# ETH3D/badslam

Measured on AMD Instinct MI355X. Metric: BA iterations/sec (and ms/iter) at N keyframes x M surfels, 640x480, higher is better.
Workload: dtype f32

## Files before the change

badslam_amd/capi.py:

```python
import ctypes as C
import os

_HERE = os.path.dirname(os.path.abspath(__file__))
LIB_PATH = os.path.join(os.environ.get("BADSLAM_LIB_DIR") or os.path.join(_HERE, "lib"), "libbadslam_hip.so")

SURFEL_ATTRIBUTE_COUNT = 17
MERGE_BUFFER_COUNT = 3
KF_ACTIVE, KF_COVISIBLE_ACTIVE, KF_INACTIVE = 0, 1, 2
ARITHMETIC_EXACT, ARITHMETIC_FAST = 0, 1

SURFEL_X, SURFEL_Y, SURFEL_Z, SURFEL_NORMAL, SURFEL_RADIUS_SQUARED, SURFEL_COLOR, SURFEL_DESCRIPTOR1, SURFEL_DESCRIPTOR2 = range(8)
SURFEL_ACCUM0 = 8


class BackendError(RuntimeError):
    pass


class Camera(C.Structure):
    _fields_ = [("fx", C.c_float), ("fy", C.c_float), ("cx", C.c_float), ("cy", C.c_float),
                ("width", C.c_int32), ("height", C.c_int32)]


class DepthParams(C.Structure):
# ... 170 lines not shown
                                            C.POINTER(Cost)]),
    "bahip_debug_set_cost_shape": (C.c_int, [C.c_int, C.c_int, C.c_int, C.c_int]),
    "bahip_debug_evaluate_pairs": (C.c_int, [C.c_void_p, C.POINTER(Frame), C.POINTER(C.c_float), C.POINTER(Surfels),
                                             C.POINTER(C.c_uint32), C.c_int, C.POINTER(C.c_float)]),
    "bahip_debug_read_pcg_vector": (C.c_int, [C.c_void_p, C.c_int, C.c_size_t, C.c_size_t, C.POINTER(C.c_float)]),
    "bahip_gather_surfel_shards": (C.c_int, [C.c_void_p, C.POINTER(Surfels), C.c_uint32, C.c_int, C.c_int, C.c_uint32, C.POINTER(Surfels),
                                             C.POINTER(C.c_uint32), C.POINTER(C.c_uint32)]),
    "bahip_extract_surfel_shard": (C.c_int, [C.c_void_p, C.POINTER(Surfels), C.c_int, C.c_int, C.c_uint32, C.POINTER(Surfels), C.POINTER(C.c_uint32)]),
    "bahip_debug_set_intrinsics_bin_capacity": (C.c_int, [C.c_void_p, C.c_int]),
    "bahip_debug_intrinsics_bin_stats": (C.c_int, [C.c_void_p, C.POINTER(C.c_uint32), C.POINTER(C.c_uint32), C.POINTER(C.c_uint64)]),
    "bahip_debug_set_intrinsics_slices": (C.c_int, [C.c_void_p, C.c_int]),
    "bahip_debug_read_intrinsics_sums": (C.c_int, [C.c_void_p, C.POINTER(C.c_float), C.POINTER(C.c_float)]),
    "bahip_exchange_stats": (C.c_int, [C.c_void_p, C.POINTER(C.c_longlong), C.POINTER(C.c_longlong), C.c_int]),
    "bahip_context_set_lifecycle_dealing": (C.c_int, [C.c_void_p, C.c_int]),
    "bahip_debug_lifecycle_deal_stats": (C.c_int, [C.c_void_p, C.POINTER(C.c_longlong), C.c_int]),
    "bahip_debug_exact_sum": (C.c_int, [C.c_void_p, C.POINTER(C.c_float), C.c_size_t, C.c_int, C.POINTER(C.c_double)]),
    "bahip_debug_count_pairs": (C.c_int, [C.c_void_p, C.POINTER(Surfels), C.POINTER(C.c_uint64)]),
    "bahip_debug_set_launch_shapes": (C.c_int, [C.c_int, C.c_int]),
    "bahip_debug_set_pose_form": (C.c_int, [C.c_int]),
    "bahip_debug_set_append_groups": (C.c_int, [C.c_int]),
    "bahip_debug_geometry_hybrid_launches": (C.c_int, [C.POINTER(C.c_longlong)]),
    "bahip_debug_set_creation_chain": (C.c_int, [C.c_int]),
    "bahip_debug_creation_chain_batches": (C.c_int, [C.POINTER(C.c_longlong)]),
    "bahip_debug_set_merge_cells": (C.c_int, [C.c_int]),
    "bahip_debug_merge_cells_batches": (C.c_int, [C.POINTER(C.c_longlong)]),
    "bahip_debug_set_pose_lds_items": (C.c_int, [C.c_int]),
    "bahip_debug_set_pose_lds_shape": (C.c_int, [C.c_int, C.c_int]),
    "bahip_debug_set_fused_iteration_begin": (C.c_int, [C.c_int]),
    "bahip_debug_set_intrinsics_reduce_form": (C.c_int, [C.c_int]),
    "bahip_debug_set_pose_rounds_ahead": (C.c_int, [C.c_int]),
    "bahip_debug_set_device_loop": (C.c_int, [C.c_int]),
    "bahip_debug_alternating_loop_calls": (C.c_int, [C.POINTER(C.c_longlong), C.POINTER(C.c_longlong)]),
    "bahip_debug_set_pcg_lds_form": (C.c_int, [C.c_int]),
    "bahip_debug_pose_form_launches": (C.c_int, [C.POINTER(C.c_longlong), C.POINTER(C.c_longlong), C.c_int]),
    "bahip_debug_pose_kernel_dispatches": (C.c_int, [C.POINTER(C.c_longlong)]),
    "bahip_debug_pcg_step1_form_launches": (C.c_int, [C.POINTER(C.c_longlong), C.POINTER(C.c_longlong)]),
    "bahip_debug_pose_limbs": (C.c_int, [C.c_void_p, C.POINTER(C.c_float), C.c_size_t, C.POINTER(C.c_longlong)]),
    "bahip_debug_jacobian": (C.c_int, [C.c_void_p, C.c_int, C.POINTER(C.c_float), C.c_int, C.POINTER(C.c_float), C.c_int]),
    "bahip_debug_read_pattern": (C.c_int, [C.c_void_p, C.c_size_t, C.c_int, C.c_int]),
    "bahip_debug_exact_math": (C.c_int, [C.c_void_p, C.c_int, C.POINTER(C.c_float), C.POINTER(C.c_float), C.c_size_t]),
    "bahip_debug_pose_step": (C.c_int, [C.c_void_p, C.POINTER(C.c_float), C.POINTER(C.c_float), C.POINTER(C.c_float)]),
    "bahip_debug_wave_reduce": (C.c_int, [C.c_void_p, C.POINTER(C.c_float), C.POINTER(C.c_float)]),
    "bahip_last_stage_time_ms": (C.c_int, [C.c_void_p, C.c_int, C.POINTER(C.c_float), C.POINTER(C.c_int)]),
    "bahip_set_profiling": (C.c_int, [C.c_void_p, C.c_int]),
    "bahip_frame_planes_create": (C.c_int, [C.c_void_p, C.c_int, C.c_int, C.c_int, C.c_int, C.POINTER(C.c_void_p)]),
    "bahip_frame_planes_update": (C.c_int, [C.c_void_p, C.c_void_p, C.POINTER(Frame)]),
    "bahip_frame_planes_destroy": (None, [C.c_void_p]),
    "bahip_stage_work_units": (C.c_int, [C.c_void_p, C.c_int, C.POINTER(C.c_longlong)]),
}

_lib = None


def load():
    global _lib
    if _lib is None:
        if not os.path.exists(LIB_PATH):
            raise BackendError(
                f"{LIB_PATH} not found: build the HIP extension first (python -c 'import __graft_entry__ as g; g.build()'). "
                "There is no CPU fallback.")
        lib = C.CDLL(LIB_PATH)
        for name, (restype, argtypes) in SIGNATURES.items():
            if os.environ.get("BADSLAM_LIB_DIR") and not hasattr(lib, name):
                continue
            fn = getattr(lib, name)
            fn.restype = restype
# ... 9 lines not shown
```

badslam_amd/csrc/ba_launch.h:

```cpp
#pragma once

#include "ba_device.h"
#include <cstdlib>

inline int bahip_env_int(const char* name, int fallback) {
  const char* e = std::getenv(name);
  return e ? std::atoi(e) : fallback;
}

#ifdef BAHIP_FAST_MATH
#define BAHIP_FLAVOUR fast
#else
#define BAHIP_FLAVOUR exact
#endif
#define BAHIP_FLAVOURED_BEGIN namespace bahip { namespace BAHIP_FLAVOUR {
#define BAHIP_FLAVOURED_END } }

namespace bahip {

struct SupportingView {
  uint32_t* b[BAHIP_MERGE_BUFFER_COUNT];
  uint32_t pitch;
};

// ... 49 lines not shown
bool launch_tile_order(hipStream_t stream, uint32_t* tile_cost, uint32_t padded_tiles, uint32_t* sched);
struct PoseLoopControl {
  int* ctl = nullptr;
  int* host_ctl = nullptr;
  int phase_end = 0;
  int iteration = 0;
  int min_iterations = 0;
  int* round_log = nullptr;
  int log_slot = 0;
  int publish = 1;
  int next_mode = -1;
  const uint8_t* in_window = nullptr;
  const int* covis_offsets = nullptr;
  const int* covis_indices = nullptr;
};
void launch_pose_solve(hipStream_t stream, void* work, int num_work, HbFixed* Hb, KfEntry* frames, int write_back,
                       int update_activation, int round, void* host_out,
                       int sequence ,
                       const PoseLoopControl* loop = nullptr);
void launch_pose_init_from_keyframes(hipStream_t stream, const KfEntry* frames, int num_kfs, void* work, HbFixed* Hb, void* host_out,
                                     int kf_rank = 0, int kf_world = 1 ,
                                     const int* stop = nullptr);

void launch_window_activation(hipStream_t stream, KfEntry* frames, int num_kfs, const uint8_t* in_window, const int* offsets,
                              const int* indices, const int* stop = nullptr);
void launch_propagate_covisible(hipStream_t stream, KfEntry* frames, int num_kfs, const int* offsets, const int* indices,
                                const int* stop = nullptr);
bool launch_iteration_begin(hipStream_t stream, KfEntry* frames, int num_kfs, int mode, const uint8_t* in_window, const int* offsets, const int* indices,
                            void* work, HbFixed* Hb, void* host_out, const int* stop);

void set_tile_waves(int waves);
long long geometry_hybrid_launches();
void set_pose_lds_waves(int waves);
void set_pose_lds_parts_shift(int shift);
void set_pose_lds_items(int items);
void pcg_step1_form_launches(long long out[2]);
long long pose_kernel_dispatches();
void pose_form_launches(long long out[2], bool reset);
void set_pose_form(int form);
void set_pose_parts(int parts);
void launch_jacobian_debug(hipStream_t stream, int kind, const float* in, float* out);
void launch_pose_step_debug(hipStream_t stream, const float* in, float* out);
void launch_exact_math_debug(hipStream_t stream, int kind, const float* in, float* out, size_t n);
void launch_pose_limbs_debug(hipStream_t stream, const float* in, long long* out, size_t n);
void launch_wave_reduce_debug(hipStream_t stream, const float* in, float* out);
void launch_evaluate_pairs(hipStream_t stream, const Intrinsics& in, const KfEntry& frame, const SurfelsView& s,
                           const uint32_t* indices, int count, float* out);

struct IntrBins {
  uint32_t* cursors;
  uint32_t* records;
  uint32_t capacity;
  int bins_x;
};
int intrinsics_bin_count(const Intrinsics& in, int* bins_x_out);
size_t intrinsics_bin_record_bytes();
void launch_intrinsics_accumulate(hipStream_t st, bool depth, bool color, const Intrinsics& in, const KfEntry* kfs, int num_kfs,
                                  const SurfelsView& s, double* glob, double* cells, const IntrBins& bins, const uint32_t* sched,
                                  uint32_t position_begin = 0, uint32_t position_count = 0 ,
                                  int classes = 1 ,
                                  int kf_rank = 0, int kf_world = 1 );
uint32_t intrinsics_sweep_positions(uint32_t surfels, const uint32_t* sched);
void launch_intrinsics_bin_reduce(hipStream_t st, bool depth, const Intrinsics& in, const SurfelsView& s, double* cells, const IntrBins& bins);
void set_intrinsics_reduce_form(int form);
size_t intrinsics_schur_partials(int S);
void launch_intrinsics_finish(hipStream_t st, bool schur, int S, const double* glob_d, const double* cells_d, float* glob_f, float* cells_f,
// ... 140 lines not shown
void launch_delete_unpack(hipStream_t st, const SurfelsView& s, const void* packed);
void launch_shard_to_cloud(hipStream_t st, const SurfelsView& shard, const SurfelsView& cloud, uint32_t rank, uint32_t world, uint32_t chunk);
void launch_cloud_to_shard(hipStream_t st, const SurfelsView& cloud, const SurfelsView& shard, uint32_t rank, uint32_t world, uint32_t chunk);
size_t sort_scratch_bytes(uint32_t n);
hipError_t sort_surfels_spatially(hipStream_t st, const SurfelsView& s, float inv_cell, void* scratch, size_t scratch_bytes);
size_t scan_temp_bytes(size_t n);
hipError_t scan_flags_inclusive(hipStream_t st, void* temp, size_t temp_bytes, const uint8_t* flags, uint32_t* out, int n);
hipError_t scan_u32_exclusive(hipStream_t st, void* temp, size_t temp_bytes, const uint32_t* in, uint32_t* out, int n);
hipError_t launch_compact(hipStream_t st, const SurfelsView& s, uint32_t* invalid, uint32_t* free_rank, uint32_t* free_list,
                          uint32_t surfel_count, void* temp, size_t temp_bytes);


#define BAHIP_FLAVOURED_DECLARATIONS                                                                                                          \
                                                                                                                      \
  void launch_activation(hipStream_t stream, const Intrinsics& in, const KfEntry* kfs, int num_kfs, const SurfelsView& s, uint32_t surfels_size); \
  void launch_normals(hipStream_t stream, const Intrinsics& in, const KfEntry* kfs, int num_kfs, const SurfelsView& s);                       \
  void launch_geometry(hipStream_t stream, bool use_depth, bool use_desc, const Intrinsics& in, const KfEntry* kfs, int num_kfs,              \
                       const SurfelsView& s, long long activate_count, const uint32_t* sched, const int* stop);                              \
  void launch_geometry_phase(hipStream_t stream, int phase, bool use_depth, bool use_desc, const Intrinsics& in, const KfEntry* kfs,          \
                             int num_kfs, const SurfelsView& s, long long activate_count, const ClassPartials& cpn, const ClassPartials& cpp); \
  void launch_activation_hits(hipStream_t stream, const Intrinsics& in, const KfEntry* kfs, int num_kfs, const SurfelsView& s,                \
                              uint32_t surfels_size, int kf_rank, int kf_world, uint32_t* hits);                                              \
  void launch_normals_phase(hipStream_t stream, int phase, const Intrinsics& in, const KfEntry* kfs, int num_kfs, const SurfelsView& s,      \
                            const ClassPartials& cp);                                                                                         \
  void set_tile_waves(int waves);                                                                                                             \
  long long geometry_hybrid_launches();                                                                                                       \
                                                                                                                        \
  void launch_pose_accumulate(hipStream_t stream, bool use_depth, bool use_desc, const Intrinsics& in, const KfEntry* frames,                 \
                              const void* work, int num_work, const SurfelsView& s, HbFixed* Hb, void* tile_bounds, bool stored_bounds,       \
                              int num_listed, uint32_t* tile_counters, int* parity_inout, uint32_t* tile_cost, const uint32_t* sched,         \
                              const int* listed_count, const int* stop);                                                                      \
  bool pose_round_can_be_queued_ahead(uint32_t surfels, int num_items, bool have_tile_counters);                                              \
  void set_pose_lds_waves(int waves);                                                                                                         \
  void set_pose_lds_parts_shift(int shift);                                                                                                   \
  void set_pose_lds_items(int items);                                                                                                         \
  long long pose_kernel_dispatches();                                                                                                         \
  void pose_form_launches(long long out[2], bool reset);                                                                                      \
  void set_pose_form(int form);                                                                                                               \
  void set_pose_parts(int parts);                                                                                                             \
  void launch_evaluate_pairs(hipStream_t stream, const Intrinsics& in, const KfEntry& frame, const SurfelsView& s, const uint32_t* indices,   \
                             int count, float* out);                                                                                          \
                                                                                                                  \
  void launch_intrinsics_accumulate(hipStream_t st, bool depth, bool color, const Intrinsics& in, const KfEntry* kfs, int num_kfs,            \
                                    const SurfelsView& s, double* glob, double* cells, const IntrBins& bins, const uint32_t* sched,           \
                                    uint32_t position_begin, uint32_t position_count, int classes, int kf_rank, int kf_world);                \
                                                                                                                         \
  void launch_pcg_init(hipStream_t st, const PcgLayout& L, const PcgExact& ex, const Intrinsics& in, const KfEntry* kfs, int num_kfs,         \
                       const SurfelsView& s, float* r, float* M, uint32_t* tile_cost, const uint32_t* sched, const PcgClasses* classes);      \
  void launch_pcg_step1(hipStream_t st, const PcgLayout& L, const PcgExact& ex, const Intrinsics& in, const KfEntry* kfs, int num_kfs,        \
                        const SurfelsView& s, const float* p, float* g, const void* ctl, const uint32_t* sched, uint32_t* tile_counters,      \
                        int* parity_inout, const PcgClasses* classes);                                                                        \
  void set_pcg_lds_form(int mode);                                                                                                            \
  void pcg_step1_form_launches(long long out[2]);                                                                                             \
                                                                                                                  \
  void launch_pcg_window_init(hipStream_t st, const PcgLayout& L, const PcgExact& ex, const Intrinsics& in, const KfEntry* kfs,              \
                              const PcgWindow& w, const SurfelsView& s, float* r, float* M);                                                  \
  void launch_pcg_window_step1(hipStream_t st, const PcgLayout& L, const PcgExact& ex, const Intrinsics& in, const KfEntry* kfs,             \
                               const PcgWindow& w, const SurfelsView& s, const float* p, float* g, const void* ctl);
namespace exact { BAHIP_FLAVOURED_DECLARATIONS }
namespace fast { BAHIP_FLAVOURED_DECLARATIONS }
#define BAHIP_PICK(in, call) do { if ((in).fast_math) fast::call; else exact::call; } while (0)

constexpr int kCostCellWords = 9;
constexpr int kCostWords = 3 * kCostCellWords + 3;
constexpr int kCostDepthCountWord = 3 * kCostCellWords, kCostPairCountWord = kCostDepthCountWord + 1, kCostFlagWord = kCostDepthCountWord + 2;
constexpr int kCostMaxWaves = 8;
// ... 18 lines not shown
```

badslam_amd/csrc/capi_debug.hip:

```cpp
#include "capi_internal.h"

using namespace bahip;
using namespace bahip_capi;

extern "C" {
int bahip_debug_evaluate_pairs(bahip_context* ctx, const bahip_frame* frame, const float frame_T_global[12],
                               const bahip_surfels* surfels, const uint32_t* surfel_indices_host, int count, float* out_host) {
  REQUIRE(ctx->have_intrinsics, "bahip_set_intrinsics not called");
  if (count <= 0) return 0;
  KfEntry e;
  if (make_entry(ctx, *frame, 0, &e)) return 1;
  memcpy(e.pose.F, frame_T_global, 12 * sizeof(float));
  DevMem idx, out;
  HIP_TRY(hipMalloc(&idx.p, sizeof(uint32_t) * count));
  HIP_TRY(hipMalloc(&out.p, sizeof(float) * 40 * count));
  HIP_TRY(hipMemcpy(idx.p, surfel_indices_host, sizeof(uint32_t) * count, hipMemcpyHostToDevice));
  launch_evaluate_pairs(ctx->stream, ctx->in, e, make_view(surfels), idx.as<uint32_t>(), count, out.as<float>());
  CHECK_LAUNCH();
  HIP_TRY(hipStreamSynchronize(ctx->stream));
  HIP_TRY(hipMemcpy(out_host, out.p, sizeof(float) * 40 * count, hipMemcpyDeviceToHost));
  return 0;
}

int bahip_debug_exact_sum(bahip_context* ctx, const float* values_host, size_t count, int mode, double* out_host) {
// ... 23 lines not shown
  if (items < 0) return fail("bahip_debug_set_pose_lds_items: items must be >= 0", __FILE__, __LINE__, hipSuccess);
  set_pose_lds_items(items);
  return 0;
}
int bahip_debug_set_pose_lds_shape(int waves, int parts_shift) {
  if (waves < 0 || waves > 16 || parts_shift < -1 || parts_shift > 3) return fail("bahip_debug_set_pose_lds_shape: waves 0 .. 16, parts_shift -1 .. 3", __FILE__, __LINE__, hipSuccess);
  set_pose_lds_waves(waves);
  set_pose_lds_parts_shift(parts_shift);
  return 0;
}
int bahip_debug_set_intrinsics_reduce_form(int form) {
  if (form < -1 || form > 1) return fail("bahip_debug_set_intrinsics_reduce_form: 0, 1 or -1 (the default)", __FILE__, __LINE__, hipSuccess);
  set_intrinsics_reduce_form(form);
  return 0;
}

int bahip_debug_set_fused_iteration_begin(int enabled) {
  g_fused_iteration_begin = enabled ? 1 : 0;
  return 0;
}

int bahip_debug_set_pose_rounds_ahead(int rounds) {
  if (rounds < 0 || rounds > BAHIP_MAX_POSE_ITERATIONS) return fail("bahip_debug_set_pose_rounds_ahead: 0 .. BAHIP_MAX_POSE_ITERATIONS", __FILE__, __LINE__, hipSuccess);
  g_pose_rounds_ahead = rounds;
  return 0;
}
int bahip_debug_pose_form_launches(long long* global_form, long long* lds_form, int reset) {
  long long n[2];
  pose_form_launches(n, reset != 0);
  if (global_form) *global_form = n[0];
  if (lds_form) *lds_form = n[1];
  return 0;
}
int bahip_debug_pcg_step1_form_launches(long long* tile_form, long long* lds_form) {
  long long n[2];
  pcg_step1_form_launches(n);
  if (tile_form) *tile_form = n[0];
  if (lds_form) *lds_form = n[1];
  return 0;
}
int bahip_debug_pose_kernel_dispatches(long long* dispatches_out) {
  if (dispatches_out) *dispatches_out = pose_kernel_dispatches();
  return 0;
}
int bahip_debug_read_tile_schedule(bahip_context* ctx, uint32_t* padded_tiles_out, uint32_t* words_out, size_t max_words) {
  HIP_TRY(hipStreamSynchronize(ctx->stream));
  *padded_tiles_out = ctx->tile_order_tiles;
  if (ctx->tile_order_tiles == 0 || words_out == nullptr) return 0;
  const size_t words = std::min(max_words, tile_schedule_words(ctx->tile_order_tiles));
  HIP_TRY(hipMemcpy(words_out, ctx->dev_tile_order, sizeof(uint32_t) * words, hipMemcpyDeviceToHost));
  return 0;
}

int bahip_debug_set_tile_order(int enabled) {
  g_tile_order_enabled = enabled ? 1 : 0;
  return 0;
}

int bahip_debug_set_append_groups(int groups) {
  REQUIRE(groups >= 0, "bahip_debug_set_append_groups: groups must be >= 0");
  set_append_groups_limit(groups);
  return 0;
}

int bahip_debug_set_pose_form(int form) {
  REQUIRE(form == 0 || form == 1 || form == 2, "pose form must be 0 (automatic), 1 (one tile per wavefront, global atomics) or 2 (persistent, LDS table)");
// ... 145 lines not shown
```

badslam_amd/csrc/kernels_pose.hip:

```cpp
#include <stdlib.h>

#include "ba_device.h"
#include <cstdio>
#include "ba_launch.h"
#include "se3_device.h"
#include "wave_cull.h"
#include "wave_reduce.h"

namespace bahip {
#ifndef BAHIP_WAVES_ATTR
#define BAHIP_WAVES_ATTR __attribute__((amdgpu_waves_per_eu(4)))
#endif
constexpr int kPoseBlock = 64;
__host__ __device__ inline int* pose_invalid_word(HbFixed* Hb) { return reinterpret_cast<int*>(Hb + 27 * kHbLimbs); }
}

BAHIP_FLAVOURED_BEGIN

__device__ __forceinline__ void accumulate_jtj(float (&acc)[28], const float (&J)[6], float wgt, float raw) {
  int q = 0;
#pragma unroll
  for (int row = 0; row < 6; ++row) {
    const float wj = wgt * J[row];
#pragma unroll
// ... 65 lines not shown
    if (pending_item >= 0 && holds_total) {
      const HbMagnitudes m = hb_split_magnitudes(pending);
      const uint32_t address = lane_offset + (uint32_t)pending_item * (uint32_t)(kHbStride * sizeof(HbFixed));
      auto* cell = reinterpret_cast<__attribute__((address_space(3))) HbFixed*>(address);
      const HbFixed lo = (HbFixed)(unsigned long long)m.lo, hi = (HbFixed)(((unsigned long long)m.hi_hi << 32) | m.hi_lo);
      if (m.valid) {
        if (m.negative) {
          if (lo) __hip_atomic_fetch_sub(cell, lo, __ATOMIC_RELAXED, __HIP_MEMORY_SCOPE_WORKGROUP);
          if (hi) __hip_atomic_fetch_sub(cell + 1, hi, __ATOMIC_RELAXED, __HIP_MEMORY_SCOPE_WORKGROUP);
        } else {
          if (lo) __hip_atomic_fetch_add(cell, lo, __ATOMIC_RELAXED, __HIP_MEMORY_SCOPE_WORKGROUP);
          if (hi) __hip_atomic_fetch_add(cell + 1, hi, __ATOMIC_RELAXED, __HIP_MEMORY_SCOPE_WORKGROUP);
        }
      } else {
        atomicOr(invalid, 1);
      }
    }
    pending_item = -1;
  }
  __device__ __forceinline__ void gathers_done() { flush(); }
  __device__ __forceinline__ void add(int item, int , float total) {
    pending = total; pending_item = item;
#ifndef BAHIP_LDS_DEFERRED
    flush();
#endif
  }
  __device__ __forceinline__ void finish() { flush(); }
};

template <bool kUseDepth, bool kUseDesc, typename Sink>
__device__ __forceinline__ void pose_tile(const Intrinsics& in, const KfEntry* __restrict__ frames, const PoseWork* __restrict__ work,
                                          int num_work, const SurfelsView& s, WaveBounds* __restrict__ tile_bounds, int stored_bounds,
                                          int num_listed, uint32_t tile, int parts, int part, Sink& sink, uint32_t* __restrict__ tile_cost,
                                          int item_begin = 0, int item_count = -1) {
  const int lane = threadIdx.x & 63;
  const int* __restrict__ listed = reinterpret_cast<const int*>(work + num_work + kPoseTailRecords) + item_begin;
  const int num_items = item_count >= 0 ? item_count : (stored_bounds ? num_listed : num_work);
  auto work_item_of = [&](int item) { return stored_bounds ? load_global(listed + item) : item_begin + item; };
  WaveBounds wb;
  if (stored_bounds) {
    wb = tile_bounds[tile];
    if (wb.r < 0.f) return;
    bool any = false;
    for (int base = part; base < num_items && !any; base += 64 * parts) {
      const int item = base + lane * parts;
      bool sees = false;
      if (item < num_items) {
        float f[12];
        load_candidate(work[work_item_of(item)].F, nullptr, f, nullptr);
        sees = sphere_may_project(in, f, wb);
      }
      any = __any(sees) != 0;
    }
    if (!any) return;
  }
  const uint32_t i = tile * kPoseBlock + lane;
  const bool in_range = i < s.size;
  const uint32_t ii = in_range ? i : 0;
  const Vec3 gp = surfel_position(s, ii);
  const Vec3 gn = surfel_normal(s, ii);
  float radius_sq = 0, d1 = 0, d2 = 0;
  if (kUseDesc) {
    radius_sq = s.row(kSurfelRadiusSquared)[ii];
    d1 = s.row(kSurfelDescriptor1)[ii];
    d2 = s.row(kSurfelDescriptor2)[ii];
  }
  const TangentPoints tp = surfel_tangent_points(gp, gn, radius_sq);

  if (!stored_bounds) {
    wb = wave_bounds(gp, in_range && (gp.x == gp.x));
    if (part == 0 && lane == 0) tile_bounds[tile] = wb;
  }
  int my_w = 0;
#ifdef BAHIP_TILE_TIMELINE
  uint32_t with_association = 0;
#endif
// ... 97 lines not shown
}

template <bool kUseDepth, bool kUseDesc>
__global__ void __launch_bounds__(kPoseBlock) BAHIP_WAVES_ATTR
pose_accumulate_kernel(Intrinsics in, const KfEntry* __restrict__ frames, const PoseWork* __restrict__ work,
                       int num_work, SurfelsView s, HbFixed* __restrict__ Hb, WaveBounds* __restrict__ tile_bounds, int stored_bounds,
                       int num_listed, int* __restrict__ invalid ,
                       uint32_t* __restrict__ tile_cost, const uint32_t* __restrict__ sched,
                       const int* __restrict__ listed_count ,
                       const int* __restrict__ stop ) {
  const int lane = threadIdx.x & 63;
  if (stop && __builtin_amdgcn_readfirstlane(load_global(stop)) != 0) return;
  if (listed_count) {
    num_listed = __builtin_amdgcn_readfirstlane(load_global(listed_count));
    if (num_listed == 0) return;
  }
  const int slot = wave_reduce28_slot(lane);
  GlobalSink sink{Hb, invalid, 0.f, -1, (slot >= 0 && slot < 27) ? slot * kHbLimbs * (int)sizeof(HbFixed) : -1};
  uint32_t tile;
  if (!scheduled_tile(blockIdx.x, gridDim.x - (sched ? kHeavySlots : 0u), sched, &tile)) return;
  pose_tile<kUseDepth, kUseDesc>(in, frames, work, num_work, s, tile_bounds, stored_bounds, num_listed, tile, (int)gridDim.y, (int)blockIdx.y, sink,
                                 tile_cost);
}

#ifndef BAHIP_POSE_LDS_WAVES
#define BAHIP_POSE_LDS_WAVES 16
#endif
constexpr int kPoseLdsWaves = BAHIP_POSE_LDS_WAVES;
#ifndef BAHIP_POSE_BATCH
#define BAHIP_POSE_BATCH 32
#endif
constexpr uint32_t kPoseBatch = BAHIP_POSE_BATCH;
constexpr int kPoseShortList = 16;
template <bool kUseDepth, bool kUseDesc, bool kSlice>
__global__ void __launch_bounds__(64 * kPoseLdsWaves) BAHIP_WAVES_ATTR
pose_accumulate_lds_kernel(Intrinsics in, const KfEntry* __restrict__ frames, const PoseWork* __restrict__ work,
                           int num_work, SurfelsView s, HbFixed* __restrict__ Hb, WaveBounds* __restrict__ tile_bounds, int stored_bounds,
                           int num_listed, int* __restrict__ invalid, uint32_t padded_tiles, uint32_t* __restrict__ tile_counters, int parity,
                           int slice_begin, int slice_count, uint32_t* __restrict__ tile_cost, const uint32_t* __restrict__ sched,
                           const int* __restrict__ listed_count ,
                           uint32_t parts_shift ,
                           const int* __restrict__ stop ) {
  extern __shared__ HbFixed table[];
  const int lane = threadIdx.x & 63;
  if (blockIdx.x == 0 && threadIdx.x < 8) tile_counters[(parity ^ 1) * 8 + threadIdx.x] = 0;
  if (stop && __builtin_amdgcn_readfirstlane(load_global(stop)) != 0) return;
  if (listed_count) {
    num_listed = __builtin_amdgcn_readfirstlane(load_global(listed_count));
    if (num_listed == 0) return;
  }
  const int item_begin = kSlice ? slice_begin : 0;
  const int num_items = kSlice ? slice_count : (stored_bounds ? num_listed : num_work);
  unsigned long long& batch_state = *reinterpret_cast<unsigned long long*>(table + (size_t)num_items * kHbStride);
  const uint32_t xcd = blockIdx.x & 7u, per_xcd = (sched_positions(padded_tiles, sched) >> 3) << parts_shift;
  uint32_t* counter = tile_counters + parity * 8 + xcd;
  for (int e = threadIdx.x; e < num_items * kHbStride; e += blockDim.x) table[e] = 0;
  const bool short_list = !kSlice && stored_bounds && num_listed <= kPoseShortList;
  if (threadIdx.x == 0 && !short_list) batch_state = ((unsigned long long)atomicAdd(counter, kPoseBatch) << 32) | ((unsigned long long)kPoseBatch << 24);
  __syncthreads();
  const int slot = wave_reduce28_slot(lane);
  const uint32_t table_address = (uint32_t)(uintptr_t)(__attribute__((address_space(3))) HbFixed*)table;
  LdsSink sink{table_address + (uint32_t)(slot > 0 ? slot : 0) * (uint32_t)(kHbLimbs * sizeof(HbFixed)), invalid, slot >= 0 && slot < 27, 0.f, -1};
  const uint32_t positions = sched_positions(padded_tiles, sched), static_stride = gridDim.x * (blockDim.x >> 6);
  uint32_t static_position = blockIdx.x * (blockDim.x >> 6) + (threadIdx.x >> 6);
  for (;;) {
    uint32_t tile = 0, position = 0;
    int parts = 1, part = 0;
    bool have_tile = false;
    if (short_list) {
      if (static_position >= positions) break;
      position = static_position;
      static_position += static_stride;
      have_tile = scheduled_tile(position, padded_tiles, sched, &tile);
    } else {
      unsigned long long taken = 0;
      if (lane == 0) taken = atomicAdd(&batch_state, 1ull);
      const uint32_t first = __builtin_amdgcn_readfirstlane((uint32_t)(taken >> 32));
      const uint32_t size = __builtin_amdgcn_readfirstlane((uint32_t)taken >> 24);
      const uint32_t index = __builtin_amdgcn_readfirstlane((uint32_t)taken & 0xffffffu);
      if (first >= per_xcd) break;
      if (index < size) {
        const uint32_t unit = first + index;
        position = (unit >> parts_shift) * 8u + xcd;
        parts = 1 << parts_shift;
        part = (int)(unit & ((1u << parts_shift) - 1u));
        have_tile = unit < per_xcd && scheduled_tile(position, padded_tiles, sched, &tile);
      } else if (index == size) {
        if (lane == 0) {
          const uint32_t left = per_xcd > first + size ? per_xcd - (first + size) : 0u;
          const uint32_t want = min(kPoseBatch, max(2u, left / (4u * (gridDim.x >> 3))));
          const uint32_t next = atomicAdd(counter, want);
          __hip_atomic_store(&batch_state, ((unsigned long long)next << 32) | ((unsigned long long)want << 24), __ATOMIC_RELAXED, __HIP_MEMORY_SCOPE_WORKGROUP);
        }
      } else {
        while ((uint32_t)(__hip_atomic_load(&batch_state, __ATOMIC_RELAXED, __HIP_MEMORY_SCOPE_WORKGROUP) >> 32) == first)
          __builtin_amdgcn_s_sleep(8);
      }
    }
    if (have_tile) {
#ifdef BAHIP_TILE_TIMELINE
      const unsigned long long t0 = wall_clock64();
#endif
      pose_tile<kUseDepth, kUseDesc>(in, frames, work, num_work, s, tile_bounds, stored_bounds, num_listed, tile, parts, part, sink, tile_cost,
                                     item_begin, kSlice ? num_items : -1);
#ifdef BAHIP_TILE_TIMELINE
      if (!stored_bounds && lane == 0 && position < 65536 && tile < 65536) {
        g_pose_timeline[position][0] = t0; g_pose_timeline[position][1] = wall_clock64(); g_pose_timeline[position][2] = tile;
        g_pose_timeline[position][3] = ((unsigned long long)g_pose_tile_stats[tile][0] << 32) | g_pose_tile_stats[tile][1];
      }
#endif
    }
  }
  __syncthreads();
  const int* __restrict__ listed = reinterpret_cast<const int*>(work + num_work + kPoseTailRecords);
  for (int e = threadIdx.x; e < num_items * kHbStride; e += blockDim.x) {
    const HbFixed v = table[e];
    if (v != 0) {
      const int item = e / kHbStride;
      const int w = stored_bounds ? listed[item_begin + item] : item_begin + item;
      __hip_atomic_fetch_add(&Hb[(size_t)w * kHbStride + (e - item * kHbStride)], v, __ATOMIC_RELAXED, __HIP_MEMORY_SCOPE_AGENT);
    }
  }
}

static int g_forced_pose_parts = bahip_env_int("BAHIP_POSE_PARTS", 0);
void set_pose_parts(int parts) { g_forced_pose_parts = parts; }


static int g_forced_pose_form = bahip_env_int("BAHIP_POSE_FORM", 0);
void set_pose_form(int form) { g_forced_pose_form = form; }
static int g_pose_lds_items = 0;
void set_pose_lds_items(int items) { g_pose_lds_items = items; }
static long long g_pose_form_launches[2] = {0, 0};
void pose_form_launches(long long out[2], bool reset) {
  out[0] = g_pose_form_launches[0]; out[1] = g_pose_form_launches[1];
  if (reset) g_pose_form_launches[0] = g_pose_form_launches[1] = 0;
}
static long long g_pose_kernel_dispatches = 0;
long long pose_kernel_dispatches() { return g_pose_kernel_dispatches; }
constexpr size_t kPoseLdsTableLimit = 128 * 1024;
#ifndef BAHIP_POSE_LDS_MIN_TILES
#define BAHIP_POSE_LDS_MIN_TILES 2048
#endif
constexpr unsigned kPoseLdsMinTiles = BAHIP_POSE_LDS_MIN_TILES;
static int g_pose_lds_parts_shift = bahip_env_int("BAHIP_POSE_LDS_PARTS_SHIFT", -1);
void set_pose_lds_parts_shift(int shift) { g_pose_lds_parts_shift = (shift >= 0 && shift <= 3) ? shift : -1; }

static int g_pose_lds_waves = 0;
void set_pose_lds_waves(int waves) { g_pose_lds_waves = (waves >= 1 && waves <= kPoseLdsWaves) ? waves : 0; }

struct PoseLdsDevice { int compute_units = 0; bool raised[8] = {}; bool failed[8] = {}; };
static PoseLdsDevice& pose_lds_device() {
  static PoseLdsDevice devices[64];
  int dev = 0;
  if (hipGetDevice(&dev) != hipSuccess || dev < 0 || dev >= 64) dev = 0;
  PoseLdsDevice& d = devices[dev];
  if (d.compute_units == 0) {
    int cus = 0;
    if (hipDeviceGetAttribute(&cus, hipDeviceAttributeMultiprocessorCount, dev) != hipSuccess || cus <= 0) cus = 256;
    d.compute_units = cus;
  }
  return d;
}

template <bool kUseDepth, bool kUseDesc, bool kSlice>
static bool launch_pose_lds(hipStream_t stream, const Intrinsics& in, const KfEntry* frames, const PoseWork* pw, int num_work,
                            const SurfelsView& s, HbFixed* Hb, WaveBounds* tb, int sb, int num_listed, unsigned tiles, size_t table_bytes,
                            uint32_t* tile_counters, int parity, int slice_begin, int slice_count, uint32_t* tile_cost, const uint32_t* sched,
                            const int* listed_count, uint32_t parts_shift, const int* stop) {
  int* invalid = pose_invalid_word(Hb);
  PoseLdsDevice& device = pose_lds_device();
  constexpr int variant = (kUseDepth ? 1 : 0) + (kUseDesc ? 2 : 0) + (kSlice ? 4 : 0);
  if (!device.raised[variant] && !device.failed[variant]) {
    if (hipFuncSetAttribute(reinterpret_cast<const void*>(&pose_accumulate_lds_kernel<kUseDepth, kUseDesc, kSlice>),
                            hipFuncAttributeMaxDynamicSharedMemorySize, (int)kPoseLdsTableLimit) == hipSuccess) device.raised[variant] = true;
    else { device.failed[variant] = true; (void)hipGetLastError(); }
  }
  if (device.failed[variant] && table_bytes + sizeof(HbFixed) > 64 * 1024) return false;
  const int waves = g_pose_lds_waves > 0 ? g_pose_lds_waves : kPoseLdsWaves;
  const unsigned units = sched_positions(tiles, sched) << parts_shift;
  const unsigned grid = std::max(8u, std::min((unsigned)device.compute_units, ((units + waves - 1) / waves + 7u) & ~7u));
  ++g_pose_kernel_dispatches;
  hipLaunchKernelGGL((pose_accumulate_lds_kernel<kUseDepth, kUseDesc, kSlice>), dim3(grid), dim3(64 * waves), table_bytes + sizeof(HbFixed) , stream, in, frames,
                     pw, num_work, s, Hb, tb, sb, num_listed, invalid, tiles, tile_counters, parity, slice_begin, slice_count, tile_cost, sched, listed_count, parts_shift, stop);
  return true;
}
template <bool kSlice>
static bool launch_pose_lds_any(bool use_depth, bool use_desc, hipStream_t stream, const Intrinsics& in, const KfEntry* frames, const PoseWork* pw,
                                int num_work, const SurfelsView& s, HbFixed* Hb, WaveBounds* tb, int sb, int num_listed, unsigned tiles,
                                size_t table_bytes, uint32_t* tile_counters, int parity, int slice_begin, int slice_count, uint32_t* tile_cost,
                                const uint32_t* sched, const int* listed_count, uint32_t parts_shift, const int* stop) {
  if (use_depth && use_desc) return launch_pose_lds<true, true, kSlice>(stream, in, frames, pw, num_work, s, Hb, tb, sb, num_listed, tiles, table_bytes, tile_counters, parity, slice_begin, slice_count, tile_cost, sched, listed_count, parts_shift, stop);
  if (use_depth) return launch_pose_lds<true, false, kSlice>(stream, in, frames, pw, num_work, s, Hb, tb, sb, num_listed, tiles, table_bytes, tile_counters, parity, slice_begin, slice_count, tile_cost, sched, listed_count, parts_shift, stop);
  return launch_pose_lds<false, true, kSlice>(stream, in, frames, pw, num_work, s, Hb, tb, sb, num_listed, tiles, table_bytes, tile_counters, parity, slice_begin, slice_count, tile_cost, sched, listed_count, parts_shift, stop);
}

bool pose_round_can_be_queued_ahead(uint32_t , int num_items, bool ) {
  const size_t item_bytes = sizeof(HbFixed) * kHbStride;
  const int per_launch = g_pose_lds_items > 0 ? std::min(g_pose_lds_items, (int)(kPoseLdsTableLimit / item_bytes)) : (int)(kPoseLdsTableLimit / item_bytes);
  return num_items <= per_launch;
}

void launch_pose_accumulate(hipStream_t stream, bool use_depth, bool use_desc, const Intrinsics& in, const KfEntry* frames,
                            const void* work, int num_work, const SurfelsView& s, HbFixed* Hb, void* tile_bounds, bool stored_bounds,
                            int num_listed, uint32_t* tile_counters, int* parity_inout, uint32_t* tile_cost, const uint32_t* sched,
                            const int* listed_count, const int* stop) {
  if (s.size == 0 || num_work == 0) return;
  const unsigned tiles = xcd_padded_tiles((s.size + kPoseBlock - 1) / kPoseBlock);
  const int forced = g_forced_pose_parts;
  const unsigned parts = (forced == 1 || forced == 2 || forced == 4 || forced == 8) ? (unsigned)forced
                         : tiles >= 32768 ? 1 : tiles >= 8192 ? 2 : 4;
  const PoseWork* pw = static_cast<const PoseWork*>(work);
  WaveBounds* tb = static_cast<WaveBounds*>(tile_bounds);
  const int sb = stored_bounds ? 1 : 0;
  const int num_items = stored_bounds ? num_listed : num_work;
  const size_t item_bytes = sizeof(HbFixed) * kHbStride;
  const bool lds_form = tile_counters != nullptr && (g_forced_pose_form == 2 || (g_forced_pose_form == 0 && tiles >= kPoseLdsMinTiles && forced == 0));
// ... 537 lines not shown
  PoseLoopControl plain = loop ? *loop : PoseLoopControl{};
  plain.next_mode = -1;
  hipLaunchKernelGGL(pose_solve_kernel, dim3((num_work + 63) / 64), dim3(64), 0, stream, static_cast<PoseWork*>(work),
                     num_work, Hb, frames, write_back, update_activation, round, static_cast<PoseWork*>(host_out), sequence, plain);
}

void launch_pose_init_from_keyframes(hipStream_t stream, const KfEntry* frames, int num_kfs, void* work, HbFixed* Hb, void* host_out,
                                     int kf_rank, int kf_world, const int* stop) {
  if (num_kfs == 0) return;
  const uint32_t mask = (uint32_t)(kf_world - 1), rank = (uint32_t)kf_rank;
  if (num_kfs <= 1024)
    hipLaunchKernelGGL(pose_init_from_keyframes_kernel<true>, dim3(1), dim3(1024), 0, stream, frames, num_kfs,
                       static_cast<PoseWork*>(work), Hb, static_cast<PoseWork*>(host_out), mask, rank, stop);
  else
    hipLaunchKernelGGL(pose_init_from_keyframes_kernel<false>, dim3((num_kfs + 63) / 64), dim3(64), 0, stream, frames, num_kfs,
                       static_cast<PoseWork*>(work), Hb, static_cast<PoseWork*>(host_out), mask, rank, stop);
}

void launch_pose_accumulate(hipStream_t stream, bool use_depth, bool use_desc, const Intrinsics& in, const KfEntry* frames,
                            const void* work, int num_work, const SurfelsView& s, HbFixed* Hb, void* tile_bounds, bool stored_bounds,
                            int num_listed, uint32_t* tile_counters, int* parity_inout, uint32_t* tile_cost, const uint32_t* sched,
                            const int* listed_count, const int* stop) {
  BAHIP_PICK(in, launch_pose_accumulate(stream, use_depth, use_desc, in, frames, work, num_work, s, Hb, tile_bounds, stored_bounds, num_listed,
                                        tile_counters, parity_inout, tile_cost, sched, listed_count, stop));
}
bool pose_round_can_be_queued_ahead(uint32_t surfels, int num_items, bool have_tile_counters) {
  return exact::pose_round_can_be_queued_ahead(surfels, num_items, have_tile_counters);
}
void set_pose_parts(int parts) { exact::set_pose_parts(parts); fast::set_pose_parts(parts); }
void set_pose_form(int form) { exact::set_pose_form(form); fast::set_pose_form(form); }
void set_pose_lds_items(int items) { exact::set_pose_lds_items(items); fast::set_pose_lds_items(items); }
void set_pose_lds_parts_shift(int shift) { exact::set_pose_lds_parts_shift(shift); fast::set_pose_lds_parts_shift(shift); }
void set_pose_lds_waves(int waves) { exact::set_pose_lds_waves(waves); fast::set_pose_lds_waves(waves); }
long long pose_kernel_dispatches() { return exact::pose_kernel_dispatches() + fast::pose_kernel_dispatches(); }
void pose_form_launches(long long out[2], bool reset) {
  long long a[2], b[2];
  exact::pose_form_launches(a, reset); fast::pose_form_launches(b, reset);
  out[0] = a[0] + b[0]; out[1] = a[1] + b[1];
}
#ifdef BAHIP_COUNT_CANDIDATES
void pose_counters_dump() { exact::pose_counters_dump(); }
#endif
#ifdef BAHIP_TILE_TIMELINE
void pose_timeline_dump(const char* path) { exact::pose_timeline_dump(path); }
#endif

}

#endif
BAHIP_FLAVOURED_BEGIN
__global__ void evaluate_pairs_kernel(Intrinsics in, KfEntry frame, SurfelsView s, const uint32_t* __restrict__ indices,
                                      int count, float* __restrict__ out) {
  const int t = blockIdx.x * blockDim.x + threadIdx.x;
  if (t >= count) return;
  float* o = out + 40 * (size_t)t;
  for (int c = 0; c < 40; ++c) o[c] = 0.f;
  const uint32_t i = indices[t];
  if (i >= s.size) return;
  const float* F = frame.pose.F;
  const Vec3 gp = surfel_position(s, i);
  const Vec3 gn = surfel_normal(s, i);
  Assoc r;
  if (!project_associate<false>(in, F, frame.geom, gp, gn, &r, nullptr)) return;
  o[0] = 1.f; o[1] = (float)r.px; o[2] = (float)r.py; o[4] = r.depth; o[34] = r.pxx; o[35] = r.pxy;
  const float inv_std = assoc_inv_std(in, r);
  const Vec3 u = assoc_unproject(r);
// ... 94 lines not shown
```

include/badslam_hip.h:

```cpp
#ifndef BADSLAM_HIP_H_
#define BADSLAM_HIP_H_

#include <stddef.h>
#include <stdint.h>

#ifdef __cplusplus
extern "C" {
#endif

#define BAHIP_SURFEL_ATTRIBUTE_COUNT 17
#define BAHIP_MERGE_BUFFER_COUNT 3
#define BAHIP_MAX_POSE_ITERATIONS 30

enum { BAHIP_KF_ACTIVE = 0, BAHIP_KF_COVISIBLE_ACTIVE = 1, BAHIP_KF_INACTIVE = 2 };

typedef struct bahip_camera {
  float fx, fy, cx, cy;
  int32_t width, height;
} bahip_camera;

typedef struct bahip_depth_params {
  float a;
  float raw_to_float_depth;
  float baseline_fx;
// ... 227 lines not shown
  float lambda_up, lambda_down;
  float lambda_min, lambda_max;
  int max_trials;
} bahip_pcg_step_control;
int bahip_pcg_iteration_controlled(bahip_context* ctx, const bahip_pcg_options* opt, const bahip_pcg_step_control* control, int windowed,
                                   int update_normals, const bahip_surfels* surfels, float* lambda_inout, bahip_camera* out_color_camera,
                                   bahip_camera* out_depth_camera, float* out_a, int* inner_steps_out, int* num_converged_out,
                                   int have_cost_before, bahip_cost* cost_before, bahip_cost* cost_after, int* trials_out,
                                   int* accepted_out);

int bahip_debug_evaluate_pairs(bahip_context* ctx, const bahip_frame* frame, const float frame_T_global[12],
                               const bahip_surfels* surfels, const uint32_t* surfel_indices, int count, float* out);

int bahip_debug_read_pcg_vector(bahip_context* ctx, int which, size_t offset, size_t count, float* out);

int bahip_debug_exact_sum(bahip_context* ctx, const float* values, size_t count, int mode, double* out);

int bahip_debug_set_launch_shapes(int tile_waves, int pose_parts);
int bahip_debug_geometry_hybrid_launches(long long* launches_out);
int bahip_debug_set_pose_form(int form);
int bahip_debug_set_tile_order(int enabled);
int bahip_debug_read_tile_schedule(bahip_context* ctx, uint32_t* padded_tiles_out, uint32_t* words_out, size_t max_words);
int bahip_debug_set_intrinsics_bin_capacity(bahip_context* ctx, int records_per_block);
int bahip_debug_intrinsics_bin_stats(bahip_context* ctx, uint32_t* capacity_out, uint32_t* most_out, uint64_t* total_out);
int bahip_debug_read_intrinsics_sums(bahip_context* ctx, float out[34], float* cells_out);
int bahip_debug_set_intrinsics_slices(bahip_context* ctx, int slices);
int bahip_debug_set_append_groups(int groups);
int bahip_debug_set_creation_chain(int enabled);
int bahip_debug_creation_chain_batches(long long* batches_out);
int bahip_debug_set_merge_cells(int enabled);
int bahip_debug_merge_cells_batches(long long* batches_out);
int bahip_debug_set_pose_lds_items(int items);
int bahip_debug_set_pose_lds_shape(int waves, int parts_shift);
int bahip_debug_set_pose_rounds_ahead(int rounds);
int bahip_debug_set_fused_iteration_begin(int enabled);
int bahip_debug_set_intrinsics_reduce_form(int form);
int bahip_debug_set_device_loop(int enabled);
int bahip_debug_alternating_loop_calls(long long* handled_out, long long* declined_out);
int bahip_debug_set_pcg_lds_form(int mode);
int bahip_debug_pose_form_launches(long long* global_form, long long* lds_form, int reset);
int bahip_debug_pose_kernel_dispatches(long long* dispatches_out);
int bahip_debug_pcg_step1_form_launches(long long* tile_form, long long* lds_form);
int bahip_debug_pose_limbs(bahip_context* ctx, const float* values, size_t count, long long* out);
int bahip_debug_jacobian(bahip_context* ctx, int kind, const float* in, int n_in, float* out, int n_out);
int bahip_debug_wave_reduce(bahip_context* ctx, const float* in_64x28, float* out_80);
int bahip_debug_read_pattern(bahip_context* ctx, size_t bytes, int pattern, int repeats);
int bahip_debug_exact_math(bahip_context* ctx, int kind, const float* in, float* out, size_t n);
int bahip_debug_pose_step(bahip_context* ctx, const float* H21_b6, const float* global_T_frame, float* out_25);
int bahip_debug_count_pairs(bahip_context* ctx, const bahip_surfels* surfels, uint64_t* counts_out);

int bahip_last_stage_time_ms(bahip_context* ctx, int stage, float* ms_out, int* launches_out);
int bahip_set_profiling(bahip_context* ctx, int enabled);
int bahip_stage_work_units(bahip_context* ctx, int stage, long long* units_out);
int bahip_gather_surfel_shards(bahip_context* ctx, const bahip_surfels* shard, uint32_t shard_surfel_count, int rank, int world, uint32_t chunk,
                               bahip_surfels* cloud, uint32_t* cloud_surfels_size_out, uint32_t* cloud_surfel_count_out);
int bahip_extract_surfel_shard(bahip_context* ctx, const bahip_surfels* cloud, int rank, int world, uint32_t chunk, bahip_surfels* shard,
                               uint32_t* shard_surfels_size_out);

int bahip_exchange_stats(bahip_context* ctx, long long* calls_out, long long* bytes_out, int reset);

#ifdef __cplusplus
}
#endif
#endif
```

Measured before the change: 746.9.

## Prescreen pose tiles against the short item list before dispatching waves

In the LDS pose accumulation kernel's short-list path, the listed work items' frame transforms are first staged into shared memory. Each wave then tests 64 scheduled tiles at a time against those items, compacting only the tiles that may be visible into a shared survivor list that waves then draw from. Tiles whose per-tile visibility scan would find nothing are therefore skipped before the full tile routine runs, and that routine is told the tile was prescreened. The cost is extra block-wide barriers per screening round, more dynamic LDS per block (possibly lower occupancy), and a global atomic counter that is bumped on every launch.

```diff
diff --git a/badslam_amd/capi.py b/badslam_amd/capi.py
--- a/badslam_amd/capi.py
+++ b/badslam_amd/capi.py
@@ -226,6 +226,8 @@
     "bahip_debug_set_device_loop": (C.c_int, [C.c_int]),
     "bahip_debug_alternating_loop_calls": (C.c_int, [C.POINTER(C.c_longlong), C.POINTER(C.c_longlong)]),
     "bahip_debug_set_pcg_lds_form": (C.c_int, [C.c_int]),
+    "bahip_debug_set_pose_short_list": (C.c_int, [C.c_int]),
+    "bahip_debug_pose_screen_route": (C.c_int, [C.c_void_p, C.POINTER(C.c_longlong), C.POINTER(C.c_longlong), C.c_int]),
     "bahip_debug_pose_form_launches": (C.c_int, [C.POINTER(C.c_longlong), C.POINTER(C.c_longlong), C.c_int]),
     "bahip_debug_pose_kernel_dispatches": (C.c_int, [C.POINTER(C.c_longlong)]),
     "bahip_debug_pcg_step1_form_launches": (C.c_int, [C.POINTER(C.c_longlong), C.POINTER(C.c_longlong)]),
diff --git a/badslam_amd/csrc/ba_launch.h b/badslam_amd/csrc/ba_launch.h
--- a/badslam_amd/csrc/ba_launch.h
+++ b/badslam_amd/csrc/ba_launch.h
@@ -105,6 +105,8 @@
 void set_tile_waves(int waves);
 long long geometry_hybrid_launches();
 void set_pose_lds_waves(int waves);
+void set_pose_short_list(int items);
+void pose_screen_route(long long out[2], bool reset);
 void set_pose_lds_parts_shift(int shift);
 void set_pose_lds_items(int items);
 void pcg_step1_form_launches(long long out[2]);
@@ -311,6 +313,8 @@
                               const int* listed_count, const int* stop);                                                                      \
   bool pose_round_can_be_queued_ahead(uint32_t surfels, int num_items, bool have_tile_counters);                                              \
   void set_pose_lds_waves(int waves);                                                                                                         \
+  void set_pose_short_list(int items);                                                                                                        \
+  void pose_screen_route(long long out[2], bool reset);                                                                                       \
   void set_pose_lds_parts_shift(int shift);                                                                                                   \
   void set_pose_lds_items(int items);                                                                                                         \
   long long pose_kernel_dispatches();                                                                                                         \
diff --git a/badslam_amd/csrc/capi_debug.hip b/badslam_amd/csrc/capi_debug.hip
--- a/badslam_amd/csrc/capi_debug.hip
+++ b/badslam_amd/csrc/capi_debug.hip
@@ -79,6 +79,19 @@
   if (lds_form) *lds_form = n[1];
   return 0;
 }
+int bahip_debug_set_pose_short_list(int items) {
+  if (items < -1 || items > 64) return fail("bahip_debug_set_pose_short_list: 0 .. 64, or -1 (the default)", __FILE__, __LINE__, hipSuccess);
+  set_pose_short_list(items);
+  return 0;
+}
+int bahip_debug_pose_screen_route(bahip_context* ctx, long long* launches_out, long long* tiles_out, int reset) {
+  HIP_TRY(hipStreamSynchronize(ctx->stream));
+  long long n[2];
+  pose_screen_route(n, reset != 0);
+  if (launches_out) *launches_out = n[0];
+  if (tiles_out) *tiles_out = n[1];
+  return 0;
+}
 int bahip_debug_pcg_step1_form_launches(long long* tile_form, long long* lds_form) {
   long long n[2];
   pcg_step1_form_launches(n);
diff --git a/badslam_amd/csrc/kernels_pose.hip b/badslam_amd/csrc/kernels_pose.hip
--- a/badslam_amd/csrc/kernels_pose.hip
+++ b/badslam_amd/csrc/kernels_pose.hip
@@ -121,7 +121,8 @@
 __device__ __forceinline__ void pose_tile(const Intrinsics& in, const KfEntry* __restrict__ frames, const PoseWork* __restrict__ work,
                                           int num_work, const SurfelsView& s, WaveBounds* __restrict__ tile_bounds, int stored_bounds,
                                           int num_listed, uint32_t tile, int parts, int part, Sink& sink, uint32_t* __restrict__ tile_cost,
-                                          int item_begin = 0, int item_count = -1) {
+                                          int item_begin = 0, int item_count = -1,
+                                          bool prescreened = false ) {
   const int lane = threadIdx.x & 63;
   const int* __restrict__ listed = reinterpret_cast<const int*>(work + num_work + kPoseTailRecords) + item_begin;
   const int num_items = item_count >= 0 ? item_count : (stored_bounds ? num_listed : num_work);
@@ -130,7 +131,7 @@
   if (stored_bounds) {
     wb = tile_bounds[tile];
     if (wb.r < 0.f) return;
-    bool any = false;
+    bool any = prescreened;
     for (int base = part; base < num_items && !any; base += 64 * parts) {
       const int item = base + lane * parts;
       bool sees = false;
@@ -294,6 +295,10 @@
 #endif
 constexpr uint32_t kPoseBatch = BAHIP_POSE_BATCH;
 constexpr int kPoseShortList = 16;
+constexpr int kPoseScreenItems = 64;
+constexpr int kPoseScreenSurvivors = 64 * kPoseLdsWaves;
+constexpr size_t kPoseLdsTail = sizeof(HbFixed)  + 16 + sizeof(float) * 16 * kPoseScreenItems + sizeof(uint32_t) * kPoseScreenSurvivors;
+__device__ unsigned long long g_pose_screen_route[2];
 template <bool kUseDepth, bool kUseDesc, bool kSlice>
 __global__ void __launch_bounds__(64 * kPoseLdsWaves) BAHIP_WAVES_ATTR
 pose_accumulate_lds_kernel(Intrinsics in, const KfEntry* __restrict__ frames, const PoseWork* __restrict__ work,
@@ -302,8 +307,9 @@
                            int slice_begin, int slice_count, uint32_t* __restrict__ tile_cost, const uint32_t* __restrict__ sched,
                            const int* __restrict__ listed_count ,
                            uint32_t parts_shift ,
-                           const int* __restrict__ stop ) {
-  extern __shared__ HbFixed table[];
+                           const int* __restrict__ stop ,
+                           int short_list_max ) {
+  extern __shared__ __attribute__((aligned(16))) HbFixed table[];
   const int lane = threadIdx.x & 63;
   if (blockIdx.x == 0 && threadIdx.x < 8) tile_counters[(parity ^ 1) * 8 + threadIdx.x] = 0;
   if (stop && __builtin_amdgcn_readfirstlane(load_global(stop)) != 0) return;
@@ -317,23 +323,95 @@
   const uint32_t xcd = blockIdx.x & 7u, per_xcd = (sched_positions(padded_tiles, sched) >> 3) << parts_shift;
   uint32_t* counter = tile_counters + parity * 8 + xcd;
   for (int e = threadIdx.x; e < num_items * kHbStride; e += blockDim.x) table[e] = 0;
-  const bool short_list = !kSlice && stored_bounds && num_listed <= kPoseShortList;
+  const bool short_list = !kSlice && stored_bounds && num_listed <= min(short_list_max, kPoseScreenItems);
+  uint32_t* screen_count = reinterpret_cast<uint32_t*>(&batch_state + 1);
+  float* screen_items = reinterpret_cast<float*>(screen_count + 4);
+  uint32_t* screen_tiles = reinterpret_cast<uint32_t*>(screen_items + 16 * kPoseScreenItems);
+  if (short_list) {
+    if (threadIdx.x < 4) screen_count[threadIdx.x] = 0;
+    if (blockIdx.x == 0 && threadIdx.x == 0) atomicAdd(&g_pose_screen_route[0], 1ull);
+    const int* __restrict__ listed = reinterpret_cast<const int*>(work + num_work + kPoseTailRecords);
+    for (int e = threadIdx.x; e < num_listed * 16; e += blockDim.x) {
+      const int c = e & 15;
+      const PoseWork& w = work[load_global(listed + (e >> 4))];
+      float v = 0.f;
+      if (c < 12) v = load_global(w.F + c);
+      else if (c == 12) v = __int_as_float(load_global(&w.skip));
+      screen_items[e] = v;
+    }
+  }
   if (threadIdx.x == 0 && !short_list) batch_state = ((unsigned long long)atomicAdd(counter, kPoseBatch) << 32) | ((unsigned long long)kPoseBatch << 24);
   __syncthreads();
   const int slot = wave_reduce28_slot(lane);
   const uint32_t table_address = (uint32_t)(uintptr_t)(__attribute__((address_space(3))) HbFixed*)table;
   LdsSink sink{table_address + (uint32_t)(slot > 0 ? slot : 0) * (uint32_t)(kHbLimbs * sizeof(HbFixed)), invalid, slot >= 0 && slot < 27, 0.f, -1};
-  const uint32_t positions = sched_positions(padded_tiles, sched), static_stride = gridDim.x * (blockDim.x >> 6);
-  uint32_t static_position = blockIdx.x * (blockDim.x >> 6) + (threadIdx.x >> 6);
   for (;;) {
     uint32_t tile = 0, position = 0;
     int parts = 1, part = 0;
     bool have_tile = false;
     if (short_list) {
-      if (static_position >= positions) break;
-      position = static_position;
-      static_position += static_stride;
-      have_tile = scheduled_tile(position, padded_tiles, sched, &tile);
+      uint32_t drawn = 0, survivors = 0;
+      if (lane == 0) { drawn = atomicAdd(&screen_count[1], 1u); survivors = screen_count[0]; }
+      drawn = __builtin_amdgcn_readfirstlane(drawn);
+      survivors = __builtin_amdgcn_readfirstlane(survivors);
+      if (drawn < survivors) {
+        tile = __builtin_amdgcn_readfirstlane(screen_tiles[drawn]);
+        have_tile = true;
+      } else {
+        const uint32_t positions = sched_positions(padded_tiles, sched), runs = (positions + 63u) >> 6, run_stride = gridDim.x * (blockDim.x >> 6);
+        const uint32_t dealt = __builtin_amdgcn_readfirstlane(screen_count[2]);
+        if (dealt >= runs) break;
+        __syncthreads();
+        if (threadIdx.x == 0) {
+          uint32_t zero = 0;
+          asm volatile("" : "+v"(zero));
+          screen_count[0] = zero; screen_count[1] = zero; screen_count[2] = dealt + run_stride;
+        }
+        __syncthreads();
+        const uint32_t screen_run = dealt + __builtin_amdgcn_readfirstlane(threadIdx.x >> 6) * gridDim.x + blockIdx.x;
+        bool sees = false;
+        uint32_t my_tile = 0;
+        uint32_t screen_lane = (uint32_t)lane;
+        asm volatile("" : "+v"(screen_lane));
+        const uint32_t p = screen_run * 64u + screen_lane;
+        if (screen_run < runs && p < positions) {
+          bool mine = true;
+          if (sched) {
+            if (p < kHeavySlots) {
+              mine = p < load_global(sched);
+              if (mine) my_tile = load_global(sched + 8 + p);
+            } else {
+              my_tile = load_global(sched + kSchedPerm + (p - kHeavySlots));
+              mine = my_tile < padded_tiles && load_global(sched + kSchedPerm + padded_tiles + my_tile) == 0;
+            }
+          } else {
+            my_tile = xcd_run_tile(p, padded_tiles);
+          }
+          if (mine && my_tile < padded_tiles) {
+            const float4 b = *reinterpret_cast<const float4*>(tile_bounds + my_tile);
+            const WaveBounds wb{b.x, b.y, b.z, b.w};
+            if (wb.r >= 0.f) {
+#pragma unroll 1
+              for (int item = 0; item < num_listed; ++item) {
+                const float4* row = reinterpret_cast<const float4*>(screen_items + 16 * item);
+                const float4 r0 = row[0], r1 = row[1], r2 = row[2];
+                const float f[12] = {r0.x, r0.y, r0.z, r0.w, r1.x, r1.y, r1.z, r1.w, r2.x, r2.y, r2.z, r2.w};
+                const bool skip = __float_as_int(screen_items[16 * item + 12]) != 0;
+                sees = sees || (!skip && sphere_may_project(in, f, wb));
+              }
+            }
+          }
+        }
+        const unsigned long long m = __builtin_amdgcn_ballot_w64(sees);
+        if (m) {
+          uint32_t base = 0;
+          if (lane == 0) base = atomicAdd(&screen_count[0], (uint32_t)__popcll(m));
+          base = __builtin_amdgcn_readfirstlane(base);
+          if (sees) screen_tiles[base + __builtin_amdgcn_mbcnt_hi((uint32_t)(m >> 32), __builtin_amdgcn_mbcnt_lo((uint32_t)m, 0u))] = my_tile;
+        }
+        __syncthreads();
+        if (threadIdx.x == 0 && screen_count[0]) atomicAdd(&g_pose_screen_route[1], (unsigned long long)screen_count[0]);
+      }
     } else {
       unsigned long long taken = 0;
       if (lane == 0) taken = atomicAdd(&batch_state, 1ull);
@@ -364,7 +442,7 @@
       const unsigned long long t0 = wall_clock64();
 #endif
       pose_tile<kUseDepth, kUseDesc>(in, frames, work, num_work, s, tile_bounds, stored_bounds, num_listed, tile, parts, part, sink, tile_cost,
-                                     item_begin, kSlice ? num_items : -1);
+                                     item_begin, kSlice ? num_items : -1, short_list);
 #ifdef BAHIP_TILE_TIMELINE
       if (!stored_bounds && lane == 0 && position < 65536 && tile < 65536) {
         g_pose_timeline[position][0] = t0; g_pose_timeline[position][1] = wall_clock64(); g_pose_timeline[position][2] = tile;
@@ -408,6 +486,17 @@
 static int g_pose_lds_parts_shift = bahip_env_int("BAHIP_POSE_LDS_PARTS_SHIFT", -1);
 void set_pose_lds_parts_shift(int shift) { g_pose_lds_parts_shift = (shift >= 0 && shift <= 3) ? shift : -1; }
 
+static int g_pose_short_list = std::min(kPoseScreenItems, std::max(0, bahip_env_int("BAHIP_POSE_SHORT_LIST", kPoseShortList)));
+void set_pose_short_list(int items) { g_pose_short_list = (items >= 0 && items <= kPoseScreenItems) ? items : kPoseShortList; }
+void pose_screen_route(long long out[2], bool reset) {
+  unsigned long long c[2] = {0, 0};
+  if (hipMemcpyFromSymbol(c, HIP_SYMBOL(g_pose_screen_route), sizeof(c)) != hipSuccess) (void)hipGetLastError();
+  out[0] = (long long)c[0]; out[1] = (long long)c[1];
+  if (reset) {
+    const unsigned long long zero[2] = {0, 0};
+    if (hipMemcpyToSymbol(HIP_SYMBOL(g_pose_screen_route), zero, sizeof(zero)) != hipSuccess) (void)hipGetLastError();
+  }
+}
 static int g_pose_lds_waves = 0;
 void set_pose_lds_waves(int waves) { g_pose_lds_waves = (waves >= 1 && waves <= kPoseLdsWaves) ? waves : 0; }
 
@@ -435,16 +524,17 @@
   constexpr int variant = (kUseDepth ? 1 : 0) + (kUseDesc ? 2 : 0) + (kSlice ? 4 : 0);
   if (!device.raised[variant] && !device.failed[variant]) {
     if (hipFuncSetAttribute(reinterpret_cast<const void*>(&pose_accumulate_lds_kernel<kUseDepth, kUseDesc, kSlice>),
-                            hipFuncAttributeMaxDynamicSharedMemorySize, (int)kPoseLdsTableLimit) == hipSuccess) device.raised[variant] = true;
+                            hipFuncAttributeMaxDynamicSharedMemorySize, (int)(kPoseLdsTableLimit + kPoseLdsTail)) == hipSuccess) device.raised[variant] = true;
     else { device.failed[variant] = true; (void)hipGetLastError(); }
   }
-  if (device.failed[variant] && table_bytes + sizeof(HbFixed) > 64 * 1024) return false;
+  if (device.failed[variant] && table_bytes + kPoseLdsTail > 64 * 1024) return false;
   const int waves = g_pose_lds_waves > 0 ? g_pose_lds_waves : kPoseLdsWaves;
   const unsigned units = sched_positions(tiles, sched) << parts_shift;
   const unsigned grid = std::max(8u, std::min((unsigned)device.compute_units, ((units + waves - 1) / waves + 7u) & ~7u));
   ++g_pose_kernel_dispatches;
-  hipLaunchKernelGGL((pose_accumulate_lds_kernel<kUseDepth, kUseDesc, kSlice>), dim3(grid), dim3(64 * waves), table_bytes + sizeof(HbFixed) , stream, in, frames,
-                     pw, num_work, s, Hb, tb, sb, num_listed, invalid, tiles, tile_counters, parity, slice_begin, slice_count, tile_cost, sched, listed_count, parts_shift, stop);
+  hipLaunchKernelGGL((pose_accumulate_lds_kernel<kUseDepth, kUseDesc, kSlice>), dim3(grid), dim3(64 * waves), table_bytes + kPoseLdsTail , stream, in, frames,
+                     pw, num_work, s, Hb, tb, sb, num_listed, invalid, tiles, tile_counters, parity, slice_begin, slice_count, tile_cost, sched, listed_count, parts_shift, stop,
+                     g_pose_short_list);
   return true;
 }
 template <bool kSlice>
@@ -1048,6 +1138,12 @@
 void set_pose_lds_items(int items) { exact::set_pose_lds_items(items); fast::set_pose_lds_items(items); }
 void set_pose_lds_parts_shift(int shift) { exact::set_pose_lds_parts_shift(shift); fast::set_pose_lds_parts_shift(shift); }
 void set_pose_lds_waves(int waves) { exact::set_pose_lds_waves(waves); fast::set_pose_lds_waves(waves); }
+void set_pose_short_list(int items) { exact::set_pose_short_list(items); fast::set_pose_short_list(items); }
+void pose_screen_route(long long out[2], bool reset) {
+  long long a[2], b[2];
+  exact::pose_screen_route(a, reset); fast::pose_screen_route(b, reset);
+  out[0] = a[0] + b[0]; out[1] = a[1] + b[1];
+}
 long long pose_kernel_dispatches() { return exact::pose_kernel_dispatches() + fast::pose_kernel_dispatches(); }
 void pose_form_launches(long long out[2], bool reset) {
   long long a[2], b[2];
diff --git a/include/badslam_hip.h b/include/badslam_hip.h
--- a/include/badslam_hip.h
+++ b/include/badslam_hip.h
@@ -283,6 +283,8 @@
 int bahip_debug_merge_cells_batches(long long* batches_out);
 int bahip_debug_set_pose_lds_items(int items);
 int bahip_debug_set_pose_lds_shape(int waves, int parts_shift);
+int bahip_debug_set_pose_short_list(int items);
+int bahip_debug_pose_screen_route(bahip_context* ctx, long long* launches_out, long long* tiles_out, int reset);
 int bahip_debug_set_pose_rounds_ahead(int rounds);
 int bahip_debug_set_fused_iteration_begin(int enabled);
 int bahip_debug_set_intrinsics_reduce_form(int form);
```

Measured after the change: 745.4. Within noise of the previous version (-0.2%).
